# danilodjor/fault-tolerant-llm-training

Hardware: AMD Instinct MI355X
Metric: tokens/sec/GPU seq-len 2048 DP at 1/2/4/8 MI355X; checkpoint save wall-clock (s) (higher is better)
Workload: dtype bf16; 1 GPU; model=llama3-8b, global_batch=1, seq_len=2048, parallelism=dp1

## Files before the change

### csrc/kernels/gemm_w4.h

```cpp
#pragma once

#include "torch_utils.h"

#include <utility>

namespace ftw4 {


typedef int i32x4_t __attribute__((ext_vector_type(4)));

template <typename F, int... I>
__device__ __forceinline__ void sfor_impl(F&& f, std::integer_sequence<int, I...>) {
  (f(std::integral_constant<int, I>{}), ...);
}
template <int N, typename F>
__device__ __forceinline__ void sfor(F&& f) {
  sfor_impl(f, std::make_integer_sequence<int, N>{});
}

constexpr int BM = 256, BK = 64, NT = 256;
constexpr int PIECE = 1024;
constexpr int FS = 2 * PIECE;
constexpr int OPA = 32 * PIECE;
constexpr int RBA = 2 * BM;
// ... 491 lines not shown
      if (wid == 0) {
        int* fl = flags + (lane & 7);
        const bool watch = (lane & 7) < nsplit - 1;
        int v = 0;
        for (int n = 0; n < p.spin; ++n) {
          v = __hip_atomic_load(fl, __ATOMIC_RELAXED, __HIP_MEMORY_SCOPE_AGENT);
          if (__all(!watch || v != 0)) break;
          __builtin_amdgcn_s_sleep(4);
        }
        __builtin_amdgcn_fence(__ATOMIC_ACQUIRE, "agent");
        const bool miss = watch && v == 0;
        if (!miss) __hip_atomic_store(fl, 0, __ATOMIC_RELAXED, __HIP_MEMORY_SCOPE_AGENT);
        const bool any = __any(miss);
        if (lane == 0) {
          lost = any ? 1 : 0;
          if (any) __hip_atomic_fetch_add(p.err, 1, __ATOMIC_RELAXED, __HIP_MEMORY_SCOPE_AGENT);
        }
      }
      asm volatile("s_waitcnt vmcnt(0)" ::: "memory");
      __syncthreads();
      split_slot = slot - (long)ks * SLOT;
      split_lost = __builtin_amdgcn_readfirstlane(lost);
    }
  }

  barrier();
  char* wl = smem + wid * 32768;
  {
    const int lr = lane & 15, hc = lane >> 4;
#pragma unroll
    for (int i = 0; i < 8; ++i) {
      const int m = i * 16 + lr;
      float4 ps[NJ];
      if (split_slot != nullptr) {
#pragma unroll
        for (int j = 0; j < NJ; ++j) ps[j] = split_slot[(i * NJ + j) * 64];
        for (int sl = 1; sl < nsplit - 1; ++sl) {
          const float4* q = split_slot + (long)sl * (4L * 8 * NJ * 64);
#pragma unroll
          for (int j = 0; j < NJ; ++j) {
            const float4 t = q[(i * NJ + j) * 64];
            ps[j].x += t.x;
            ps[j].y += t.y;
            ps[j].z += t.z;
            ps[j].w += t.w;
          }
        }
      }
#pragma unroll
      for (int j = 0; j < NJ; ++j) {
        const int ch = 2 * j + (hc >> 1);
        f32x4_t v = acc[i][j];
        if (split_slot != nullptr) {
          v[0] = ps[j].x + v[0];
          v[1] = ps[j].y + v[1];
          v[2] = ps[j].z + v[2];
          v[3] = ps[j].w + v[3];
          if (split_lost) v = f32x4_t{__builtin_nanf(""), __builtin_nanf(""), __builtin_nanf(""), __builtin_nanf("")};
        }
        uint2 pk;
        pk.x = pk2<E>(v[0], v[1]);
        pk.y = pk2<E>(v[2], v[3]);
        *reinterpret_cast<uint2*>(wl + m * 256 + ((ch ^ (m & 15)) << 4) + (((hc ^ (m >> 3)) & 1) << 3)) = pk;
      }
    }
  }
  __builtin_amdgcn_s_waitcnt(0xc07f);
  __builtin_amdgcn_wave_barrier();
#ifdef FT_W4_PROBE
  pt3 = __builtin_amdgcn_s_memrealtime();
#endif
  const int cc = lane & 15;
  float sq = 0.f;
  if constexpr (EPI == W4_SWIGLU_BWD) {
    if (cc < 2 * NJ) {
      const int gn = n0 + wn * NW + cc * 8;
#pragma unroll
      for (int hb = 0; hb < 2; ++hb) {
        uint4 g16[16], u16[16];
#pragma unroll
        for (int q = 0; q < 16; ++q) {
          const long gm = m0 + wm * 128 + (hb * 16 + q) * 4 + (lane >> 4);
          g16[q] = *reinterpret_cast<const uint4*>(p.r + gm * p.ldr + gn);
          u16[q] = *reinterpret_cast<const uint4*>(p.r + gm * p.ldr + p.ffn + gn);
        }
#pragma unroll
        for (int q = 0; q < 16; ++q) {
          const int row = (hb * 16 + q) * 4 + (lane >> 4);
          const long gm = m0 + wm * 128 + row;
          const uint4 v = stg_swap(*reinterpret_cast<const uint4*>(wl + row * 256 + ((cc ^ (row & 15)) << 4)),
                                   (q >> 1) & 1);
          float d8[8], g8[8], u8[8], dg[8], du[8];
          unpack8e<E>(v, d8);
          unpack8e<E>(g16[q], g8);
          unpack8e<E>(u16[q], u8);
#pragma unroll
          for (int e = 0; e < 8; ++e) swiglu_grad(g8[e], u8[e], d8[e], p.exact, dg[e], du[e]);
          *reinterpret_cast<uint4*>(p.c + gm * p.ldc + gn) = pack8e<E>(dg);
          *reinterpret_cast<uint4*>(p.c + gm * p.ldc + p.ffn + gn) = pack8e<E>(du);
        }
      }
    }
  } else if (cc < 2 * NJ) {
    auto store_rows = [&](auto tail_tag) {
      constexpr bool TAIL = decltype(tail_tag)::value;
      for (int r4 = 0; r4 < 32; r4 += 4)
#pragma unroll
      for (int u = 0; u < 4; ++u) {
        const int rr = r4 + u;
        const int row = rr * 4 + (lane >> 4);
        const long gm = m0 + wm * 128 + row;
        if constexpr (TAIL) {
          if (gm >= p.M) continue;
        }
        uint4 v = stg_swap(*reinterpret_cast<const uint4*>(wl + row * 256 + ((cc ^ (row & 15)) << 4)),
                           u >> 1);
        const int gn = EPI == W4_SWIGLU ? (wn ? p.ffn : 0) + f0 + cc * 8 : n0 + wn * NW + cc * 8;
        if constexpr (EPI == W4_RES) {
          float a[8], r[8];
          unpack8e<E>(v, a);
          unpack8e<E>(*reinterpret_cast<const uint4*>(p.r + gm * p.ldr + gn), r);
#pragma unroll
          for (int q = 0; q < 8; ++q) a[q] += r[q];
          v = pack8e<E>(a);
        } else if constexpr (EPI == W4_ROPE) {
          if (gn < p.rope_cols) {
            const int pos = (int)(gm % p.rope_seq);
            const int i0 = (gn % p.rope_hd) >> 1;
            const float* cs = p.cos_t + (long)pos * (p.rope_hd >> 1) + i0;
            const float* sn = p.sin_t + (long)pos * (p.rope_hd >> 1) + i0;
            const float4 c4 = *reinterpret_cast<const float4*>(cs);
            const float4 s4 = *reinterpret_cast<const float4*>(sn);
            float a[8];
            unpack8e<E>(v, a);
            const float cv[4] = {c4.x, c4.y, c4.z, c4.w}, sv[4] = {s4.x, s4.y, s4.z, s4.w};
            float o[8];
#pragma unroll
            for (int q = 0; q < 4; ++q) {
              o[2 * q] = a[2 * q] * cv[q] - a[2 * q + 1] * sv[q];
              o[2 * q + 1] = a[2 * q] * sv[q] + a[2 * q + 1] * cv[q];
            }
            v = pack8e<E>(o);
          }
        }
        if (p.part != nullptr) {
          float a[8];
          unpack8e<E>(v, a);
#pragma unroll
          for (int q = 0; q < 8; ++q) sq = fmaf(a[q], a[q], sq);
        }
        if (!(p.dbg & 1)) *reinterpret_cast<uint4*>(p.c + gm * p.ldc + gn) = v;
      }
    };
    if (mtail)
      store_rows(std::true_type{});
    else
      store_rows(std::false_type{});
  }
  if (p.part != nullptr) {
    sq = wave_sum(sq);
    __syncthreads();
    float* red = reinterpret_cast<float*>(smem);
    if (lane == 0) red[wid] = sq;
    __syncthreads();
    if (tid == 0) p.part[tn * p.tiles_m + tm] = (red[0] + red[1]) + (red[2] + red[3]);
    if (tb == 0)
      for (int i = ntiles + tid; i < p.part_n; i += NT) p.part[i] = 0.f;
  }
  if constexpr (EPI == W4_SWIGLU) {
    __syncthreads();
    char* gl = smem + (wm * 2) * 32768;
    char* ul = smem + (wm * 2 + 1) * 32768;
    if (cc < 2 * NJ) {
      for (int r4 = 0; r4 < 16; r4 += 4)
#pragma unroll
      for (int u = 0; u < 4; ++u) {
        const int row = wn * 64 + (r4 + u) * 4 + (lane >> 4);
        const int off = row * 256 + ((cc ^ (row & 15)) << 4);
        const bool sw = u >> 1;
        float g8[8], u8[8], a8[8];
        unpack8e<E>(stg_swap(*reinterpret_cast<const uint4*>(gl + off), sw), g8);
        unpack8e<E>(stg_swap(*reinterpret_cast<const uint4*>(ul + off), sw), u8);
#pragma unroll
        for (int q = 0; q < 8; ++q) a8[q] = g8[q] * sigmoid_f(g8[q], p.exact) * u8[q];
        const uint4 av = pack8e<E>(a8);
        *reinterpret_cast<uint4*>(p.act + (m0 + wm * 128 + row) * (long)p.ffn + f0 + cc * 8) = av;
        *reinterpret_cast<uint4*>(gl + off) = stg_swap(av, sw);
      }
    }
    if (p.actT == nullptr) {
      probe_end();
      return;
    }
    __syncthreads();
    constexpr int CH = 2 * NJ;
    for (int k = tid; k < 2 * 16 * CH; k += NT) {
      const int fc = k % CH, tg = (k / CH) % 16, hf = k / (16 * CH);
      const char* al = smem + (hf * 2) * 32768;
      uint16_t e[8][8];
#pragma unroll
      for (int i = 0; i < 8; ++i) {
        const int row = tg * 8 + i;
        const uint4 v = stg_swap(*reinterpret_cast<const uint4*>(al + row * 256 + ((fc ^ (row & 15)) << 4)), tg & 1);
        const uint32_t wv[4] = {v.x, v.y, v.z, v.w};
#pragma unroll
        for (int q = 0; q < 4; ++q) {
          e[i][2 * q] = (uint16_t)(wv[q] & 0xffffu);
          e[i][2 * q + 1] = (uint16_t)(wv[q] >> 16);
        }
      }
      bf16_t* dst = p.actT + (long)(f0 + fc * 8) * p.M + m0 + hf * 128 + tg * 8;
#pragma unroll
      for (int j = 0; j < 8; ++j) {
        uint4 o;
        o.x = e[0][j] | ((uint32_t)e[1][j] << 16);
        o.y = e[2][j] | ((uint32_t)e[3][j] << 16);
        o.z = e[4][j] | ((uint32_t)e[5][j] << 16);
        o.w = e[6][j] | ((uint32_t)e[7][j] << 16);
        *reinterpret_cast<uint4*>(dst + (long)j * p.M) = o;
      }
    }
  }
  probe_end();
}

template <class E, int NJ, bool AT, bool BT>
void launch_nj(const W4Args& p, int epi, hipStream_t st) {
  const dim3 g(p.tiles_m * p.tiles_n * (p.splits > 1 ? p.splits : 1));
  if constexpr (!AT && !BT) {
    if (epi == W4_ROPE) {
      hipLaunchKernelGGL((gemm_w4_kernel<E, NJ, W4_ROPE, false, false>), g, dim3(NT), 0, st, p);
      return;
    }
    if (epi == W4_SWIGLU) {
      hipLaunchKernelGGL((gemm_w4_kernel<E, NJ, W4_SWIGLU, false, false>), g, dim3(NT), 0, st, p);
      return;
    }
  }
  if constexpr (!AT && BT) {
    if (epi == W4_SWIGLU_BWD) {
      hipLaunchKernelGGL((gemm_w4_kernel<E, NJ, W4_SWIGLU_BWD, false, true>), g, dim3(NT), 0, st, p);
      return;
    }
  }
  TORCH_CHECK(epi == W4_STORE || epi == W4_RES, "gemm_w4: epilogue ", epi, " not built for this layout");
  if (epi == W4_RES)
    hipLaunchKernelGGL((gemm_w4_kernel<E, NJ, W4_RES, AT, BT>), g, dim3(NT), 0, st, p);
  else
    hipLaunchKernelGGL((gemm_w4_kernel<E, NJ, W4_STORE, AT, BT>), g, dim3(NT), 0, st, p);
}

template <bool AT, bool BT>
void launch_l(at::ScalarType st_, int nj, const W4Args& p, int epi, hipStream_t st) {
  FT_DISPATCH_E16(st_, {
    switch (nj) {
      case 8: launch_nj<E, 8, AT, BT>(p, epi, st); break;
      case 7: launch_nj<E, 7, AT, BT>(p, epi, st); break;
      case 6: launch_nj<E, 6, AT, BT>(p, epi, st); break;
      default: launch_nj<E, 4, AT, BT>(p, epi, st); break;
    }
  });
}

void launch_fwd(at::ScalarType st_, int nj, const W4Args& p, int epi, hipStream_t st);
void launch_dx(at::ScalarType st_, int nj, const W4Args& p, int epi, hipStream_t st);
void launch_dw(at::ScalarType st_, int nj, const W4Args& p, int epi, hipStream_t st);

}
```

### fault_tolerant_llm_training_amd/models/llama.py

```python
from __future__ import annotations

from dataclasses import dataclass, replace
from typing import Optional

import torch
import torch.utils.checkpoint
import torch.nn as nn

from ..ops import functional as Fx
from .flat import FlatParamSpace


@dataclass
class TransformerModelArgs:

    dim: int = 4096
    n_layers: int = 32
    n_heads: int = 32
    n_kv_heads: Optional[int] = None
    multiple_of: int = 256
    ffn_dim_multiplier: Optional[float] = None
    norm_eps: float = 1e-5
    rope_theta: float = 10000
    norm_type: str = "rmsnorm"
    seq_len: int = 2048
    vocab_size: int = -1

    @property
    def kv_heads(self) -> int:
        return self.n_heads if self.n_kv_heads is None else self.n_kv_heads

    @property
    def head_dim(self) -> int:
        return self.dim // self.n_heads

    @property
    def ffn_hidden(self) -> int:
        hidden = int(2 * (4 * self.dim) / 3)
        if self.ffn_dim_multiplier is not None:
            hidden = int(self.ffn_dim_multiplier * hidden)
        return self.multiple_of * ((hidden + self.multiple_of - 1) // self.multiple_of)


PRESETS = {
    "llama3-8b": dict(dim=4096, n_layers=32, n_heads=32, n_kv_heads=8, ffn_dim_multiplier=1.3,
                      multiple_of=1024, rope_theta=500000),
    "gpt2-small": dict(dim=768, n_layers=12, n_heads=12, n_kv_heads=12, multiple_of=256,
                       rope_theta=10000),
    "gpt2-medium": dict(dim=1024, n_layers=24, n_heads=16, n_kv_heads=16, multiple_of=256,
                        rope_theta=10000),
    "tiny": dict(dim=256, n_layers=2, n_heads=4, n_kv_heads=2, multiple_of=64, rope_theta=10000),
}


def model_args_for(preset: str, vocab_size: int, seq_len: int, **overrides) -> TransformerModelArgs:
    if preset not in PRESETS:
        raise ValueError(f"unknown model preset {preset!r}; choose from {sorted(PRESETS)}")
    cfg = dict(PRESETS[preset])
    cfg.update(overrides)
    return TransformerModelArgs(vocab_size=vocab_size, seq_len=seq_len, **cfg)


def rope_tables(head_dim: int, end: int, theta: float):
    freqs = 1.0 / (theta ** (torch.arange(0, head_dim, 2)[: (head_dim // 2)].float() / head_dim))
    t = torch.arange(end, device=freqs.device)
    freqs = torch.outer(t, freqs).float()
    cis = torch.polar(torch.ones_like(freqs), freqs)
    return cis.real.contiguous(), cis.imag.contiguous()


class _Weight(nn.Module):

    def __init__(self, *shape):
        super().__init__()
        self.weight = nn.Parameter(torch.empty(*shape, device="meta"))


class Attention(nn.Module):
    def __init__(self, a: TransformerModelArgs):
        super().__init__()
        self.n_heads, self.n_kv_heads, self.head_dim = a.n_heads, a.kv_heads, a.head_dim
        self.wq = _Weight(a.n_heads * a.head_dim, a.dim)
        self.wk = _Weight(a.kv_heads * a.head_dim, a.dim)
        self.wv = _Weight(a.kv_heads * a.head_dim, a.dim)
        self.wo = _Weight(a.dim, a.n_heads * a.head_dim)
        self.wqkv = None
        self.wqkv_sink = None


class FeedForward(nn.Module):
    def __init__(self, a: TransformerModelArgs):
        super().__init__()
        h = a.ffn_hidden
        self.w1 = _Weight(h, a.dim)
        self.w2 = _Weight(a.dim, h)
        self.w3 = _Weight(h, a.dim)
        self.w13 = None
        self.w13_sink = None


class TransformerBlock(nn.Module):
    def __init__(self, layer_id: int, a: TransformerModelArgs):
        super().__init__()
        self.layer_id = layer_id
        self.attention = Attention(a)
        self.feed_forward = FeedForward(a)
        self.attention_norm = _Weight(a.dim)
        self.ffn_norm = _Weight(a.dim)
        self.eps = a.norm_eps
        self.layernorm = a.norm_type == "layernorm"
        self.attn_keep = Fx.AttentionKeep()

    def forward(self, h, d, cos, sin, seq_len, gen=None, doc=None):
        at, ff = self.attention, self.feed_forward
        sk = lambda p: getattr(p, "_ft_sink", None)
        if d is None:
            xn = Fx.norm(h, self.attention_norm.weight, sk(self.attention_norm.weight), self.eps, self.layernorm)
        else:
            h, xn = Fx.add_norm(h, d, self.attention_norm.weight, sk(self.attention_norm.weight), self.eps,
                                self.layernorm)
        o = Fx.qkv_rope_attention(xn, at.wqkv, at.wqkv_sink, cos, sin, seq_len, at.n_heads, at.n_kv_heads,
                                  at.head_dim, self.attn_keep if gen is not None else None, -1 if gen is None else gen,
                                  doc)
        da = Fx.linear(o.view(*h.shape[:-1], -1), at.wo.weight, sk(at.wo.weight))
        h, hn = Fx.add_norm(h, da, self.ffn_norm.weight, sk(self.ffn_norm.weight), self.eps, self.layernorm)
        return h, Fx.feed_forward(hn, ff.w13, ff.w2.weight, ff.w13_sink, sk(ff.w2.weight))


class Transformer(nn.Module):
    def __init__(self, model_args: TransformerModelArgs):
        super().__init__()
        a = model_args
        self.model_args = a
        self.vocab_size = a.vocab_size
        self.n_layers = a.n_layers
        self.tok_embeddings = _Weight(a.vocab_size, a.dim)
        cos, sin = rope_tables(a.head_dim, a.seq_len, a.rope_theta)
        self.register_buffer("rope_cos", cos, persistent=False)
        self.register_buffer("rope_sin", sin, persistent=False)
        self.layers = nn.ModuleDict({str(i): TransformerBlock(i, a) for i in range(a.n_layers)})
        self.norm = _Weight(a.dim)
        self.output = _Weight(a.vocab_size, a.dim)
        self.flat: Optional[FlatParamSpace] = None
        self.gate = None
        self._ranges = None
        self.recompute_layers = 0
        self.recompute_attention = False
        self._gen = 0
        self.doc_bos: Optional[int] = None

    def set_document_mask(self, bos_id: Optional[int]) -> None:
        self.doc_bos = None if bos_id is None else int(bos_id)

    def set_activation_checkpointing(self, n_layers: int, recompute_attention: bool = False) -> None:
        self.recompute_layers = self.n_layers if n_layers < 0 else min(int(n_layers), self.n_layers)
        self.recompute_attention = bool(recompute_attention)

    def flat_layout(self):
        names = ["tok_embeddings.weight"]
        for i in range(self.n_layers):
            p = f"layers.{i}."
            names += [p + "attention_norm.weight", p + "attention.wq.weight", p + "attention.wk.weight",
                      p + "attention.wv.weight", p + "attention.wo.weight", p + "ffn_norm.weight",
                      p + "feed_forward.w1.weight", p + "feed_forward.w3.weight", p + "feed_forward.w2.weight"]
        names += ["norm.weight", "output.weight"]
        return names

    def materialize(self, device, dtype=torch.bfloat16, seed: int = 1234) -> "Transformer":
        self.flat = FlatParamSpace(self, self.flat_layout(), device, dtype)
        self.rope_cos = self.rope_cos.to(device)
        self.rope_sin = self.rope_sin.to(device)
        for layer in self.layers.values():
            at, ff = layer.attention, layer.feed_forward
            i = layer.layer_id
            at.wqkv, at.wqkv_sink = self.flat.fused(
                [f"layers.{i}.attention.wq.weight", f"layers.{i}.attention.wk.weight", f"layers.{i}.attention.wv.weight"])
            ff.w13, ff.w13_sink = self.flat.fused(
                [f"layers.{i}.feed_forward.w1.weight", f"layers.{i}.feed_forward.w3.weight"])
        self._ranges = self._param_ranges()
        self.init_weights(seed)
        return self

    def _param_ranges(self):
        sl = self.flat.slots

        def span(prefix):
            ss = [s for n, s in sl.items() if n.startswith(prefix)]
            return min(s.offset for s in ss), max(s.offset + s.numel for s in ss)

        emb = span("tok_embeddings.")
        layers = [span(f"layers.{i}.") for i in range(self.n_layers)]
        lo_n, hi_n = span("norm.")
        lo_o, hi_o = span("output.")
        return emb, layers, (min(lo_n, lo_o), max(hi_n, hi_o))

    def _wait(self, rng):
        if self.gate is not None:
            self.gate.wait(*rng)

    @torch.no_grad()
    def init_weights(self, seed: int = 1234):
        dev = self.flat.device
        gen = torch.Generator(device=dev)
        for idx, (name, p) in enumerate(self.named_parameters()):
            gen.manual_seed(seed * 1000003 + idx)
            if name == "tok_embeddings.weight":
                p.normal_(0.0, 1.0, generator=gen)
            elif p.dim() == 1:
                p.fill_(1.0)
            else:
                bound = 1.0 / (p.shape[1] ** 0.5)
                p.uniform_(-bound, bound, generator=gen)

    def sinks_in_backward_order(self):
        out = []
        for layer in self.layers.values():
            out += [layer.attention.wqkv_sink, layer.feed_forward.w13_sink]
        return out

    def forward(self, tokens: torch.Tensor, labels: Optional[torch.Tensor] = None,
                inv_count: Optional[torch.Tensor] = None):
        B, S = tokens.shape
        sk = lambda p: getattr(p, "_ft_sink", None)
        emb_r, layer_r, final_r = self._ranges
        self._wait(emb_r)
        h = Fx.embedding(tokens, self.tok_embeddings.weight, sk(self.tok_embeddings.weight))
        cos, sin = self.rope_cos, self.rope_sin
        doc = None if self.doc_bos is None else Fx.doc_bounds(tokens, self.doc_bos)
        d = None
        self._gen += 1
        gen = None if self.recompute_attention else self._gen
        for i, layer in enumerate(self.layers.values()):
            self._wait(layer_r[i])
            if i < self.recompute_layers and torch.is_grad_enabled():
                h, d = torch.utils.checkpoint.checkpoint(layer, h, d, cos, sin, S, gen, doc, use_reentrant=False)
            else:
                h, d = layer(h, d, cos, sin, S, None, doc)
        self._wait(final_r)
        a = self.model_args
        ln = a.norm_type == "layernorm"
        if d is None:
            h = Fx.norm(h, self.norm.weight, sk(self.norm.weight), a.norm_eps, ln)
        else:
            _, h = Fx.add_norm(h, d, self.norm.weight, sk(self.norm.weight), a.norm_eps, ln)
        if labels is None:
            return Fx.linear(h, self.output.weight, sk(self.output.weight))
        if inv_count is None:
            n = (labels != Fx.IGNORE_INDEX).sum().clamp(min=1)
            inv_count = (1.0 / n.float()).to(h.device)
        return Fx.lm_head_cross_entropy(h, self.output.weight, labels, inv_count, sk(self.output.weight))

    @torch.no_grad()
    def evaluate(self, tokens: torch.Tensor, labels: torch.Tensor, acc: torch.Tensor) -> torch.Tensor:
        B, S = tokens.shape
        emb_r, layer_r, final_r = self._ranges
        self._wait(emb_r)
        h = Fx.embedding(tokens, self.tok_embeddings.weight, None)
        cos, sin = self.rope_cos, self.rope_sin
        doc = None if self.doc_bos is None else Fx.doc_bounds(tokens, self.doc_bos)
        d = None
        self._gen += 1
        for i, layer in enumerate(self.layers.values()):
            self._wait(layer_r[i])
            h, d = layer(h, d, cos, sin, S, None, doc)
        self._wait(final_r)
        a = self.model_args
        ln = a.norm_type == "layernorm"
        if d is None:
            h = Fx.norm(h, self.norm.weight, None, a.norm_eps, ln)
        else:
            _, h = Fx.add_norm(h, d, self.norm.weight, None, a.norm_eps, ln)
        return Fx.lm_head_eval(h, self.output.weight, labels, acc)

    def num_params(self) -> int:
        return sum(p.numel() for p in self.parameters())


def build_model(args: TransformerModelArgs, device, dtype=torch.bfloat16, seed: int = 1234) -> Transformer:
    return Transformer(args).materialize(device, dtype, seed)


PEAK_FLOPS = {torch.bfloat16: 2.5e15, torch.float16: 2.5e15, torch.float32: 157.3e12, torch.float64: 78.6e12}


def flops_per_token(a: TransformerModelArgs, seq_len: int) -> float:
    d, L, hd = a.dim, a.n_layers, a.head_dim
    per_layer = d * (a.n_heads * hd) + 2 * d * (a.kv_heads * hd) + (a.n_heads * hd) * d + 3 * d * a.ffn_hidden
    n_mm = L * per_layer + d * a.vocab_size
    attn = L * 2 * 2 * seq_len * a.n_heads * hd / 2
    return 6 * n_mm + 3 * attn
```

### fault_tolerant_llm_training_amd/ops/functional.py

```python
from __future__ import annotations

import collections
import functools
import os
from typing import Optional

import torch
import torch.nn.functional as F

from .._native import kernels, native
from .grad_sink import GradSink

IGNORE_INDEX = -100

_BLAS_ONLY = os.environ.get("FT_GEMM_BLAS", "0") == "1"
_W4_FWD = True
_W4_BWD = os.environ.get("FT_W4_BWD", "1") != "0"
_W4_DTYPES = (torch.bfloat16, torch.float16)
_F32_MFMA = os.environ.get("FT_F32_MFMA", "1") != "0"


def set_f32_mfma(on: bool) -> None:
    global _F32_MFMA
    _F32_MFMA = bool(on)
# ... 201 lines not shown
        ctx.wshape = weight.shape
        if native(weight):
            return kernels().embedding_fwd(tokens.contiguous(), weight)
        return F.embedding(tokens, weight)

    @staticmethod
    def backward(ctx, dy):
        (tokens,) = ctx.saved_tensors
        sink = ctx.sink
        dy = dy.contiguous()
        if sink is not None and sink.gather is not None:
            if sink.defer:
                sink.stash.append((tokens.reshape(-1), dy.reshape(-1, dy.shape[-1])))
                return None, None, None
            if sink.stash:
                tokens = torch.cat([t for t, _ in sink.stash] + [tokens.reshape(-1)])
                dy = torch.cat([g for _, g in sink.stash] + [dy.reshape(-1, dy.shape[-1])])
                sink.stash = []
            tokens, dy = sink.gather(tokens, dy)
        if native(dy):
            if sink is None:
                dw = torch.zeros(ctx.wshape, dtype=dy.dtype, device=dy.device)
                kernels().embedding_bwd_(dy, tokens.contiguous(), dw, False)
                return None, dw, None
            part = sink.part if (sink.part is not None and not sink.accumulate) else None
            kernels().embedding_bwd_(dy, tokens.contiguous(), sink.buf, sink.accumulate, part)
            if part is not None:
                sink.sq_done = True
            sink.ready()
            return None, None, None
        dw = torch.zeros(ctx.wshape, dtype=torch.float32, device=dy.device)
        if dy.is_cuda:
            dw.index_put_((tokens.reshape(-1),), dy.reshape(-1, ctx.wshape[1]).float(), accumulate=True)
        else:
            dw.index_add_(0, tokens.reshape(-1), dy.reshape(-1, ctx.wshape[1]).float())
        return None, _write_weight_grad(sink, dw.to(dy.dtype)), None


def embedding(tokens, weight, sink=None):
    return EmbeddingFn.apply(tokens, weight, sink)


def norm_reference(x: torch.Tensor, w: torch.Tensor, eps: float, layernorm: bool) -> torch.Tensor:
    xf = x.float()
    if layernorm:
        xf = xf - xf.mean(-1, keepdim=True)
    n = xf * torch.rsqrt(xf.pow(2).mean(-1, keepdim=True) + eps)
    return n.type_as(x) * w


class NormFn(torch.autograd.Function):
    @staticmethod
    def forward(ctx, x, weight, sink, eps, layernorm):
        ctx.sink, ctx.eps, ctx.ln = sink, eps, layernorm
        if native(x):
            xc = x.contiguous()
            y, rstd, mean = kernels().norm_fwd(xc, weight, eps, layernorm)
            ctx.save_for_backward(xc, weight, rstd, mean)
            return y
        ctx.save_for_backward(x, weight)
        return norm_reference(x, weight, eps, layernorm)

    @staticmethod
    def backward(ctx, dy):
        sink = ctx.sink
        if native(dy):
            x, w, rstd, mean = ctx.saved_tensors
            if sink is not None:
                return norm_bwd_into_sink(dy.contiguous(), x, w, rstd, mean, sink), None, None, None, None
            dw = torch.empty_like(w)
            dx = kernels().norm_bwd(dy.contiguous(), x, w, rstd, mean, dw, None, False)
            return dx, dw, None, None, None
        x, w = ctx.saved_tensors
        with torch.enable_grad():
            xr = x.detach().requires_grad_(True)
            wr = w.detach().requires_grad_(True)
            y = norm_reference(xr, wr, ctx.eps, ctx.ln)
            dx, dw = torch.autograd.grad(y, (xr, wr), dy)
        return dx, _write_weight_grad(sink, dw), None, None, None


def norm(x, weight, sink=None, eps: float = 1e-5, layernorm: bool = False):
    return NormFn.apply(x, weight, sink, eps, layernorm)


class AddNormFn(torch.autograd.Function):

    @staticmethod
    def forward(ctx, x, d, weight, sink, eps, layernorm):
        ctx.sink, ctx.eps, ctx.ln = sink, eps, layernorm
        if native(x):
            y, rstd, mean, h = kernels().add_norm_fwd(x.contiguous(), d.contiguous(), weight, eps, layernorm)
            ctx.save_for_backward(h, weight, rstd, mean)
            return h, y
        h = x + d
        ctx.save_for_backward(h, weight)
        return h, norm_reference(h, weight, eps, layernorm)

    @staticmethod
    def backward(ctx, dh, dy):
        sink = ctx.sink
        if native(dy):
            h, w, rstd, mean = ctx.saved_tensors
            dres = dh.contiguous() if dh is not None else None
            if sink is not None:
                g = norm_bwd_into_sink(dy.contiguous(), h, w, rstd, mean, sink, dres)
                return g, g, None, None, None, None
            buf = torch.empty_like(w)
            g = kernels().norm_bwd(dy.contiguous(), h, w, rstd, mean, buf, dres, False)
            return g, g, buf, None, None, None
        h, w = ctx.saved_tensors
        with torch.enable_grad():
            hr = h.detach().requires_grad_(True)
            wr = w.detach().requires_grad_(True)
            y = norm_reference(hr, wr, ctx.eps, ctx.ln)
            g, dw = torch.autograd.grad(y, (hr, wr), dy)
        if dh is not None:
            g = g + dh
        return g, g, _write_weight_grad(sink, dw), None, None, None


def add_norm(x, d, weight, sink=None, eps: float = 1e-5, layernorm: bool = False):
    return AddNormFn.apply(x, d, weight, sink, eps, layernorm)


class LinearFn(torch.autograd.Function):
    @staticmethod
    def forward(ctx, x, weight, sink, residual):
        K = x.shape[-1]
        N = weight.shape[0]
        x2 = x.reshape(-1, K)
        y = mm_fwd(x2, weight, residual)
        ctx.sink = sink
        ctx.has_res = residual is not None
        ctx.xshape = x.shape
        ctx.save_for_backward(x2, weight)
        return y.view(*x.shape[:-1], N)

    @staticmethod
    def backward(ctx, dy):
        x2, w = ctx.saved_tensors
        N = w.shape[0]
        dy2 = dy.reshape(-1, N)
        dw = None
        dw = weight_grad_async(dy2, x2, ctx.sink)
        dx = mm_dx(dy2, w).view(ctx.xshape)
        return dx, dw, None, (dy if ctx.has_res else None)


def linear(x, weight, sink=None, residual=None):
    return LinearFn.apply(x, weight, sink, residual)


def swiglu_reference(gu: torch.Tensor) -> torch.Tensor:
    g, u = gu.chunk(2, dim=-1)
    return F.silu(g) * u


class SwiGLUFn(torch.autograd.Function):
    @staticmethod
    def forward(ctx, gu):
        ctx.save_for_backward(gu)
        if native(gu):
            return kernels().swiglu_fwd(gu.contiguous())
        return swiglu_reference(gu)

    @staticmethod
    def backward(ctx, da):
        (gu,) = ctx.saved_tensors
        if native(da):
            return kernels().swiglu_bwd(da.contiguous(), gu.contiguous())
        with torch.enable_grad():
            x = gu.detach().requires_grad_(True)
            (dx,) = torch.autograd.grad(swiglu_reference(x), (x,), da)
        return dx


def swiglu(gu):
    return SwiGLUFn.apply(gu)


_W4_SWIGLU = True


def set_w4_swiglu(on: bool) -> None:
    global _W4_SWIGLU
    _W4_SWIGLU = bool(on)


def _ffn_w4t_ok(x2: torch.Tensor, w13: torch.Tensor, w2: torch.Tensor) -> bool:
    if not (_W4_SWIGLU and _W4_FWD and _W4_BWD and w13.is_contiguous() and w2.is_contiguous()):
        return False
    T, D = x2.shape
    F = w2.shape[1]
    if T % 256 or D % 128:
        return False
    nj = _swiglu_nj(T, F)
    if nj == 0 or (T // 256) * (F // (16 * nj)) < _W4_MIN_WGS:
        return False
    return (w4_route(T, F, D, False, True, x2, w2) and w4_route(2 * F, D, T, True, True, x2, w13)
            and w4_route(D, F, T, True, True, x2, w2) and w4_route(T, D, 2 * F, False, True, x2, w13))


@functools.lru_cache(maxsize=64)
def _swiglu_nj(T: int, F: int) -> int:
    return int(kernels().gemm_swiglu_pick(T, F))


class FeedForwardW4Fn(torch.autograd.Function):

    @staticmethod
    def forward(ctx, x, w13, w2, sink13, sink2):
        K_ = kernels()
        D = x.shape[-1]
        x2 = x.reshape(-1, D).contiguous()
        gu, a, _ = K_.gemm_swiglu_w4(x2, w13, False)
        y = mm_fwd(a, w2)
        ctx.sinks = (sink13, sink2)
        ctx.xshape = x.shape
        ctx.save_for_backward(x2, gu, a, w13, w2)
        return y.view(*x.shape[:-1], w2.shape[0])

    @staticmethod
    def backward(ctx, dy):
        x2, gu, a, w13, w2 = ctx.saved_tensors
        sink13, sink2 = ctx.sinks
        dy2 = dy.reshape(-1, w2.shape[0]).contiguous()
        dw2 = weight_grad_async(dy2, a, sink2)
        dgu = kernels().gemm_swiglu_bwd_w4(dy2, w2, gu, 0)
        dw13 = weight_grad_async(dgu, x2, sink13)
        dx = mm_dx(dgu, w13).view(ctx.xshape)
        return dx, dw13, dw2, None, None


class FeedForwardFn(torch.autograd.Function):

    @staticmethod
    def forward(ctx, x, w13, w2, sink13, sink2):
        K_ = kernels()
        D = x.shape[-1]
        x2 = x.reshape(-1, D)
        gu = mm_fwd(x2, w13)
        a = K_.swiglu_fwd(gu)
        y = mm_fwd(a, w2)
        ctx.sinks = (sink13, sink2)
        ctx.xshape = x.shape
        ctx.save_for_backward(x2, gu, a, w13, w2)
        return y.view(*x.shape[:-1], w2.shape[0])

    @staticmethod
    def backward(ctx, dy):
        x2, gu, a, w13, w2 = ctx.saved_tensors
        sink13, sink2 = ctx.sinks
        dy2 = dy.reshape(-1, w2.shape[0]).contiguous()
        dw2 = weight_grad_async(dy2, a, sink2)
        dgu = kernels().swiglu_bwd(mm_dx(dy2, w2), gu)
        dw13 = weight_grad_async(dgu, x2, sink13)
        dx = mm_dx(dgu, w13).view(ctx.xshape)
        return dx, dw13, dw2, None, None


def feed_forward(x, w13, w2, sink13=None, sink2=None):
    if native(x):
        T, D = x.numel() // x.shape[-1], x.shape[-1]
        if _ffn_w4t_ok(x.reshape(T, D), w13, w2):
            return FeedForwardW4Fn.apply(x, w13, w2, sink13, sink2)
        return FeedForwardFn.apply(x, w13, w2, sink13, sink2)
    return linear(swiglu(linear(x, w13, sink13)), w2, sink2)


_HEAD_CHUNK_MB = float(os.environ.get("FT_HEAD_CHUNK_MB", "1024"))


def _head_rows(T: int, V: int) -> int:
    rows = int(_HEAD_CHUNK_MB * 2**20) // (2 * V)
    rows = max(256, rows // 256 * 256)
    return min(T, rows)


def _dx_into(out: torch.Tensor, dy2: torch.Tensor, w: torch.Tensor) -> None:
    mm_dx(dy2, w, out)


def _head_fwd(h2: torch.Tensor, w: torch.Tensor) -> torch.Tensor:
    return mm_fwd(h2.contiguous(), w)


class LMHeadCrossEntropyFn(torch.autograd.Function):

    @staticmethod
    def forward(ctx, h, weight, sink, labels, inv_count):
        D = h.shape[-1]
        h2 = h.reshape(-1, D)
        lab = labels.reshape(-1)
        ctx.sink = sink
        ctx.hshape = h.shape
        ctx.native = native(h)
        if not ctx.native:
            logits = torch.mm(h2, weight.t())
            loss = F.cross_entropy(logits.float(), lab, reduction="sum", ignore_index=IGNORE_INDEX) * inv_count
            ctx.save_for_backward(h2, weight, lab, inv_count)
            return loss
        K_ = kernels()
        h2 = h2.contiguous()
        lab = lab.contiguous()
        T, V = h2.shape[0], weight.shape[0]
        rows = _head_rows(T, V)
        need = ctx.needs_input_grad[0] or ctx.needs_input_grad[1] or sink is not None
        fused = need and not (sink is not None and sink.accumulate)
        ctx.fused = fused
        ctx.rows = rows
        inv = inv_count.float().reshape(1).contiguous()
        one = torch.ones(1, dtype=torch.float32, device=h.device)
        dh = torch.empty_like(h2) if fused else None
        dw = None
        if fused:
            dw = sink.buf.view(V, D) if sink is not None else torch.empty_like(weight)
        losses, lses = [], []
        for c, r0 in enumerate(range(0, T, rows)):
            hc, lc = h2[r0 : r0 + rows], lab[r0 : r0 + rows]
            logits = _head_fwd(hc, weight)
            lr, lse = K_.xent_fwd(logits, lc, IGNORE_INDEX)
            losses.append(lr)
            if fused:
                K_.xent_bwd_(logits, lc, lse, one, inv, IGNORE_INDEX)
                _dx_into(dh[r0 : r0 + rows], logits, weight)
                _dw_into(dw, logits, hc, c > 0, sink if r0 + rows >= T else None)
            else:
                lses.append(lse)
            del logits
        loss = (losses[0] if len(losses) == 1 else torch.cat(losses)).sum() * inv_count
        if fused:
            ctx.save_for_backward(dh, dw if sink is None else None)
        else:
            ctx.save_for_backward(h2, weight, lab, inv, torch.cat(lses))
        return loss

    @staticmethod
    def backward(ctx, g):
        sink = ctx.sink
        if not ctx.native:
            h2, w, lab, inv_count = ctx.saved_tensors
            with torch.enable_grad():
                hr = h2.detach().requires_grad_(True)
                wr = w.detach().requires_grad_(True)
                logits = torch.mm(hr, wr.t())
                loss = F.cross_entropy(logits.float(), lab, reduction="sum", ignore_index=IGNORE_INDEX) * inv_count
                dh, dw = torch.autograd.grad(loss, (hr, wr), g)
            return dh.view(ctx.hshape), _write_weight_grad(sink, dw), None, None, None
        K_ = kernels()
        gf = g.detach().float().reshape(1).contiguous()
        if ctx.fused:
            dh, dw = ctx.saved_tensors
            K_.scale_by_(dh, gf)
            if sink is not None:
                K_.scale_by_(sink.buf, gf)
                if sink.sq_done:
                    sink.part.mul_(gf * gf)
                sink.ready()
                return dh.view(ctx.hshape), None, None, None, None
            K_.scale_by_(dw, gf)
            return dh.view(ctx.hshape), dw, None, None, None
        h2, w, lab, inv, lse = ctx.saved_tensors
        T, D = h2.shape
        V = w.shape[0]
        rows = ctx.rows
        dh = torch.empty_like(h2)
        dw = sink.buf.view(V, D) if sink is not None else torch.empty_like(w)
        acc0 = sink.accumulate if sink is not None else False
        for c, r0 in enumerate(range(0, T, rows)):
            hc, lc = h2[r0 : r0 + rows], lab[r0 : r0 + rows]
            logits = _head_fwd(hc, w)
            K_.xent_bwd_(logits, lc, lse[r0 : r0 + rows].contiguous(), gf, inv, IGNORE_INDEX)
            _dx_into(dh[r0 : r0 + rows], logits, w)
            _dw_into(dw, logits, hc, acc0 or c > 0, sink if r0 + rows >= T else None)
            del logits
        if sink is not None:
            sink.ready()
            return dh.view(ctx.hshape), None, None, None, None
        return dh.view(ctx.hshape), dw, None, None, None


def lm_head_cross_entropy(h, weight, labels, inv_count, sink=None):
    return LMHeadCrossEntropyFn.apply(h, weight, sink, labels, inv_count)

# ... 35 lines not shown
```

### fault_tolerant_llm_training_amd/ops/routing.py

```python
from . import attention as A
from . import functional as Fx


class _Spec:

    def __init__(self, *shape, dtype, cuda=True):
        self.shape, self.dtype, self.is_cuda = tuple(shape), dtype, cuda

    def is_contiguous(self):
        return True


def _name(kernel, M, N, K, a_t, b_t):
    if kernel != "w4":
        return {"f32": "f32 mfma", "blas": "hipBLASLt"}[kernel]
    nj, sp = Fx._w4_plan(M, N, K, a_t, b_t)
    return f"w4 {32 * nj}" + (f" x{sp}" if sp > 1 else "")


def routing_table(margs, dtype, tokens: int = 2048, cuda: bool = True) -> dict:
    T, D, V = tokens, margs.dim, margs.vocab_size
    hd, Hq, Hkv, Fh = margs.head_dim, margs.n_heads, margs.kv_heads, margs.ffn_hidden
    W = (Hq + 2 * Hkv) * hd
    sp = lambda *s: _Spec(*s, dtype=dtype, cuda=cuda)
    x, wqkv, wo, w13, w2, head = sp(T, D), sp(W, D), sp(D, Hq * hd), sp(2 * Fh, D), sp(D, Fh), sp(V, D)

    def fwd(xx, w):
        return _name(Fx.fwd_kernel(xx, w), xx.shape[0], w.shape[0], xx.shape[1], False, False)

    def dx(Tn, w):
        N, K = w.shape
        return _name(Fx.dx_kernel(sp(Tn, N), w), Tn, K, N, False, True)

    def dw(Tn, w):
        N, K = w.shape
        return _name(Fx.dw_kernel(sp(Tn, N), sp(Tn, K)), N, K, Tn, True, True)

    t = {}
    t["qkv fwd"] = "w4 qkv+rope" if A._qkv_rope_ok(x, wqkv, hd) else fwd(x, wqkv)
    t["qkv dX"], t["qkv dW"] = dx(T, wqkv), dw(T, wqkv)
    t["wo fwd"], t["wo dX"], t["wo dW"] = fwd(sp(T, Hq * hd), wo), dx(T, wo), dw(T, wo)
    if cuda and Fx._ffn_w4t_ok(x, w13, w2):
        t["w13 fwd"], t["w2 dX"] = "w4 swiglu", "w4 swiglu-bwd"
    else:
        t["w13 fwd"], t["w2 dX"] = fwd(x, w13), dx(T, w2)
    t["w13 dX"], t["w13 dW"] = dx(T, w13), dw(T, w13)
    t["w2 fwd"], t["w2 dW"] = fwd(sp(T, Fh), w2), dw(T, w2)
    rows = Fx._head_rows(T, V)
    t["head fwd"], t["head dX"], t["head dW"] = fwd(sp(rows, D), head), dx(rows, head), dw(rows, head)
    return t
```

Measured before the change: 20780 tokens/s (whole job, sum over GPUs).

## Fuse residual add into W4 down-projection GEMM epilogue and hoist next-layer norm

Adds a residual-add epilogue path to the W4 GEMM store so the FFN down-projection writes h + FFN(x) directly. The block then computes the next layer's attention norm inside a fused autograd function, which removes the separate add_norm kernel and its read/write of the residual stream. The same fusion for the wo projection exists but is off by default. In exchange the forward signature and checkpointing path get more complex, and the epilogue does extra global loads of the residual per tile.

```diff
diff --git a/csrc/kernels/gemm_w4.h b/csrc/kernels/gemm_w4.h
--- a/csrc/kernels/gemm_w4.h
+++ b/csrc/kernels/gemm_w4.h
@@ -667,8 +667,42 @@
         if (!(p.dbg & 1)) *reinterpret_cast<uint4*>(p.c + gm * p.ldc + gn) = v;
       }
     };
+    auto store_rows_res = [&]() {
+      const int gn = n0 + wn * NW + cc * 8;
+#pragma unroll
+      for (int hb = 0; hb < 2; ++hb) {
+        uint4 r16[16];
+#pragma unroll
+        for (int q = 0; q < 16; ++q) {
+          const long gm = m0 + wm * 128 + (hb * 16 + q) * 4 + (lane >> 4);
+          r16[q] = *reinterpret_cast<const uint4*>(p.r + gm * p.ldr + gn);
+        }
+#pragma unroll
+        for (int q = 0; q < 16; ++q) {
+          const int row = (hb * 16 + q) * 4 + (lane >> 4);
+          const long gm = m0 + wm * 128 + row;
+          uint4 v = stg_swap(*reinterpret_cast<const uint4*>(wl + row * 256 + ((cc ^ (row & 15)) << 4)),
+                             (q >> 1) & 1);
+          float a[8], r[8];
+          unpack8e<E>(v, a);
+          unpack8e<E>(r16[q], r);
+#pragma unroll
+          for (int e = 0; e < 8; ++e) a[e] += r[e];
+          v = pack8e<E>(a);
+          if (p.part != nullptr) {
+            float s[8];
+            unpack8e<E>(v, s);
+#pragma unroll
+            for (int e = 0; e < 8; ++e) sq = fmaf(s[e], s[e], sq);
+          }
+          if (!(p.dbg & 1)) *reinterpret_cast<uint4*>(p.c + gm * p.ldc + gn) = v;
+        }
+      }
+    };
     if (mtail)
       store_rows(std::true_type{});
+    else if constexpr (EPI == W4_RES)
+      store_rows_res();
     else
       store_rows(std::false_type{});
   }
diff --git a/fault_tolerant_llm_training_amd/models/llama.py b/fault_tolerant_llm_training_amd/models/llama.py
--- a/fault_tolerant_llm_training_amd/models/llama.py
+++ b/fault_tolerant_llm_training_amd/models/llama.py
@@ -111,10 +111,12 @@
         self.layernorm = a.norm_type == "layernorm"
         self.attn_keep = Fx.AttentionKeep()
 
-    def forward(self, h, d, cos, sin, seq_len, gen=None, doc=None):
+    def forward(self, h, d, cos, sin, seq_len, gen=None, doc=None, xn=None, next_norm=None):
         at, ff = self.attention, self.feed_forward
         sk = lambda p: getattr(p, "_ft_sink", None)
-        if d is None:
+        if xn is not None:
+            pass
+        elif d is None:
             xn = Fx.norm(h, self.attention_norm.weight, sk(self.attention_norm.weight), self.eps, self.layernorm)
         else:
             h, xn = Fx.add_norm(h, d, self.attention_norm.weight, sk(self.attention_norm.weight), self.eps,
@@ -122,9 +124,18 @@
         o = Fx.qkv_rope_attention(xn, at.wqkv, at.wqkv_sink, cos, sin, seq_len, at.n_heads, at.n_kv_heads,
                                   at.head_dim, self.attn_keep if gen is not None else None, -1 if gen is None else gen,
                                   doc)
-        da = Fx.linear(o.view(*h.shape[:-1], -1), at.wo.weight, sk(at.wo.weight))
-        h, hn = Fx.add_norm(h, da, self.ffn_norm.weight, sk(self.ffn_norm.weight), self.eps, self.layernorm)
-        return h, Fx.feed_forward(hn, ff.w13, ff.w2.weight, ff.w13_sink, sk(ff.w2.weight))
+        o = o.view(*h.shape[:-1], -1)
+        if Fx.native(o) and Fx.linear_res_ok(o.view(-1, o.shape[-1]), at.wo.weight):
+            h, hn = Fx.linear_add_norm(o, at.wo.weight, h, self.ffn_norm.weight, sk(at.wo.weight),
+                                       sk(self.ffn_norm.weight), self.eps, self.layernorm)
+        else:
+            da = Fx.linear(o, at.wo.weight, sk(at.wo.weight))
+            h, hn = Fx.add_norm(h, da, self.ffn_norm.weight, sk(self.ffn_norm.weight), self.eps, self.layernorm)
+        if next_norm is not None and Fx.native(hn) and Fx.ffn_res_ok(hn.view(-1, hn.shape[-1]), ff.w13, ff.w2.weight):
+            h, xn = Fx.feed_forward_add_norm(hn, ff.w13, ff.w2.weight, h, next_norm, ff.w13_sink, sk(ff.w2.weight),
+                                             sk(next_norm), self.eps, self.layernorm)
+            return h, None, xn
+        return h, Fx.feed_forward(hn, ff.w13, ff.w2.weight, ff.w13_sink, sk(ff.w2.weight)), None
 
 
 class Transformer(nn.Module):
@@ -144,6 +155,7 @@
         self.flat: Optional[FlatParamSpace] = None
         self.gate = None
         self._ranges = None
+        self._norm_names = None
         self.recompute_layers = 0
         self.recompute_attention = False
         self._gen = 0
@@ -178,6 +190,7 @@
             ff.w13, ff.w13_sink = self.flat.fused(
                 [f"layers.{i}.feed_forward.w1.weight", f"layers.{i}.feed_forward.w3.weight"])
         self._ranges = self._param_ranges()
+        self._norm_names = [f"layers.{i}.attention_norm.weight" for i in range(self.n_layers)] + ["norm.weight"]
         self.init_weights(seed)
         return self
 
@@ -193,6 +206,14 @@
         lo_n, hi_n = span("norm.")
         lo_o, hi_o = span("output.")
         return emb, layers, (min(lo_n, lo_o), max(hi_n, hi_o))
+
+    def _next_norm(self, i, layers):
+        w = layers[i + 1].attention_norm.weight if i + 1 < len(layers) else self.norm.weight
+        if self.gate is not None and self.flat is not None:
+            s = self.flat.slots.get(self._norm_names[i + 1]) if self._norm_names else None
+            if s is not None:
+                self.gate.wait(s.offset, s.offset + s.numel)
+        return w
 
     def _wait(self, rng):
         if self.gate is not None:
@@ -227,19 +248,24 @@
         h = Fx.embedding(tokens, self.tok_embeddings.weight, sk(self.tok_embeddings.weight))
         cos, sin = self.rope_cos, self.rope_sin
         doc = None if self.doc_bos is None else Fx.doc_bounds(tokens, self.doc_bos)
-        d = None
+        d = xn = None
         self._gen += 1
         gen = None if self.recompute_attention else self._gen
-        for i, layer in enumerate(self.layers.values()):
+        layers = list(self.layers.values())
+        for i, layer in enumerate(layers):
             self._wait(layer_r[i])
+            nxt = self._next_norm(i, layers)
             if i < self.recompute_layers and torch.is_grad_enabled():
-                h, d = torch.utils.checkpoint.checkpoint(layer, h, d, cos, sin, S, gen, doc, use_reentrant=False)
+                h, d, xn = torch.utils.checkpoint.checkpoint(layer, h, d, cos, sin, S, gen, doc, xn, nxt,
+                                                             use_reentrant=False)
             else:
-                h, d = layer(h, d, cos, sin, S, None, doc)
+                h, d, xn = layer(h, d, cos, sin, S, None, doc, xn, nxt)
         self._wait(final_r)
         a = self.model_args
         ln = a.norm_type == "layernorm"
-        if d is None:
+        if xn is not None:
+            h = xn
+        elif d is None:
             h = Fx.norm(h, self.norm.weight, sk(self.norm.weight), a.norm_eps, ln)
         else:
             _, h = Fx.add_norm(h, d, self.norm.weight, sk(self.norm.weight), a.norm_eps, ln)
@@ -258,15 +284,18 @@
         h = Fx.embedding(tokens, self.tok_embeddings.weight, None)
         cos, sin = self.rope_cos, self.rope_sin
         doc = None if self.doc_bos is None else Fx.doc_bounds(tokens, self.doc_bos)
-        d = None
+        d = xn = None
         self._gen += 1
-        for i, layer in enumerate(self.layers.values()):
+        layers = list(self.layers.values())
+        for i, layer in enumerate(layers):
             self._wait(layer_r[i])
-            h, d = layer(h, d, cos, sin, S, None, doc)
+            h, d, xn = layer(h, d, cos, sin, S, None, doc, xn, self._next_norm(i, layers))
         self._wait(final_r)
         a = self.model_args
         ln = a.norm_type == "layernorm"
-        if d is None:
+        if xn is not None:
+            h = xn
+        elif d is None:
             h = Fx.norm(h, self.norm.weight, None, a.norm_eps, ln)
         else:
             _, h = Fx.add_norm(h, d, self.norm.weight, None, a.norm_eps, ln)
diff --git a/fault_tolerant_llm_training_amd/ops/functional.py b/fault_tolerant_llm_training_amd/ops/functional.py
--- a/fault_tolerant_llm_training_amd/ops/functional.py
+++ b/fault_tolerant_llm_training_amd/ops/functional.py
@@ -377,6 +377,66 @@
     return LinearFn.apply(x, weight, sink, residual)
 
 
+_W4_RESIDUAL = True
+_W4_RESIDUAL_WO = False
+
+
+def set_w4_residual(on: bool, wo: Optional[bool] = None) -> None:
+    global _W4_RESIDUAL, _W4_RESIDUAL_WO
+    _W4_RESIDUAL = bool(on)
+    if wo is not None:
+        _W4_RESIDUAL_WO = bool(wo)
+
+
+def _res_fwd_w4(T: int, N: int, K: int, x, w) -> bool:
+    return _W4_RESIDUAL and _kernel(_W4_FWD, w.is_contiguous(), T, N, K, False, False, x, w) == "w4"
+
+
+def linear_res_ok(x2, w) -> bool:
+    return _W4_RESIDUAL_WO and _res_fwd_w4(x2.shape[0], w.shape[0], x2.shape[1], x2, w)
+
+
+def ffn_res_ok(x2, w13, w2) -> bool:
+    return (x2.is_cuda and _ffn_w4t_ok(x2, w13, w2)
+            and _res_fwd_w4(x2.shape[0], w2.shape[0], w2.shape[1], x2, w2))
+
+
+def _norm_bwd_res(ctx, saved, dh, dy):
+    h1, nw, rstd, mean = saved
+    dres = dh.contiguous() if dh is not None else None
+    if ctx.norm_sink is not None:
+        return norm_bwd_into_sink(dy.contiguous(), h1, nw, rstd, mean, ctx.norm_sink, dres), None
+    buf = torch.empty_like(nw)
+    return kernels().norm_bwd(dy.contiguous(), h1, nw, rstd, mean, buf, dres, False), buf
+
+
+class LinearAddNormFn(torch.autograd.Function):
+
+    @staticmethod
+    def forward(ctx, x, weight, h, norm_w, sink, norm_sink, eps, layernorm):
+        K, N = x.shape[-1], weight.shape[0]
+        x2 = x.reshape(-1, K).contiguous()
+        h1 = kernels().gemm_nt_w4(x2, weight, None, h.reshape(-1, N).contiguous(), 0, 0).view(h.shape)
+        y, rstd, mean = kernels().norm_fwd(h1, norm_w, eps, layernorm)
+        ctx.sink, ctx.norm_sink, ctx.xshape = sink, norm_sink, x.shape
+        ctx.save_for_backward(h1, norm_w, rstd, mean, x2, weight)
+        return h1, y
+
+    @staticmethod
+    def backward(ctx, dh, dy):
+        saved = ctx.saved_tensors
+        x2, w = saved[4:]
+        g, dnw = _norm_bwd_res(ctx, saved[:4], dh, dy)
+        dy2 = g.reshape(-1, w.shape[0])
+        dw = weight_grad_async(dy2, x2, ctx.sink)
+        dx = mm_dx(dy2, w).view(ctx.xshape)
+        return dx, dw, g, dnw, None, None, None, None
+
+
+def linear_add_norm(x, weight, h, norm_w, sink=None, norm_sink=None, eps: float = 1e-5, layernorm: bool = False):
+    return LinearAddNormFn.apply(x, weight, h, norm_w, sink, norm_sink, eps, layernorm)
+
+
 def swiglu_reference(gu: torch.Tensor) -> torch.Tensor:
     g, u = gu.chunk(2, dim=-1)
     return F.silu(g) * u
@@ -456,6 +516,39 @@
         dw13 = weight_grad_async(dgu, x2, sink13)
         dx = mm_dx(dgu, w13).view(ctx.xshape)
         return dx, dw13, dw2, None, None
+
+
+class FeedForwardW4AddNormFn(torch.autograd.Function):
+
+    @staticmethod
+    def forward(ctx, x, w13, w2, h, norm_w, sink13, sink2, norm_sink, eps, layernorm):
+        K_ = kernels()
+        D = x.shape[-1]
+        x2 = x.reshape(-1, D).contiguous()
+        gu, a, _ = K_.gemm_swiglu_w4(x2, w13, False)
+        h1 = K_.gemm_nt_w4(a, w2, None, h.reshape(-1, w2.shape[0]).contiguous(), 0, 0).view(h.shape)
+        y, rstd, mean = K_.norm_fwd(h1, norm_w, eps, layernorm)
+        ctx.sinks, ctx.norm_sink, ctx.xshape = (sink13, sink2), norm_sink, x.shape
+        ctx.save_for_backward(h1, norm_w, rstd, mean, x2, gu, a, w13, w2)
+        return h1, y
+
+    @staticmethod
+    def backward(ctx, dh, dy):
+        saved = ctx.saved_tensors
+        x2, gu, a, w13, w2 = saved[4:]
+        sink13, sink2 = ctx.sinks
+        g, dnw = _norm_bwd_res(ctx, saved[:4], dh, dy)
+        dy2 = g.reshape(-1, w2.shape[0])
+        dw2 = weight_grad_async(dy2, a, sink2)
+        dgu = kernels().gemm_swiglu_bwd_w4(dy2, w2, gu, 0)
+        dw13 = weight_grad_async(dgu, x2, sink13)
+        dx = mm_dx(dgu, w13).view(ctx.xshape)
+        return dx, dw13, dw2, g, dnw, None, None, None, None, None
+
+
+def feed_forward_add_norm(x, w13, w2, h, norm_w, sink13=None, sink2=None, norm_sink=None, eps: float = 1e-5,
+                          layernorm: bool = False):
+    return FeedForwardW4AddNormFn.apply(x, w13, w2, h, norm_w, sink13, sink2, norm_sink, eps, layernorm)
 
 
 class FeedForwardFn(torch.autograd.Function):
diff --git a/fault_tolerant_llm_training_amd/ops/routing.py b/fault_tolerant_llm_training_amd/ops/routing.py
--- a/fault_tolerant_llm_training_amd/ops/routing.py
+++ b/fault_tolerant_llm_training_amd/ops/routing.py
@@ -16,6 +16,14 @@
         return {"f32": "f32 mfma", "blas": "hipBLASLt"}[kernel]
     nj, sp = Fx._w4_plan(M, N, K, a_t, b_t)
     return f"w4 {32 * nj}" + (f" x{sp}" if sp > 1 else "")
+
+
+def residual_table(margs, dtype, tokens: int = 2048, cuda: bool = True) -> dict:
+    T, D, Fh = tokens, margs.dim, margs.ffn_hidden
+    sp = lambda *s: _Spec(*s, dtype=dtype, cuda=cuda)
+    x, wo, w13, w2 = sp(T, D), sp(D, margs.n_heads * margs.head_dim), sp(2 * Fh, D), sp(D, Fh)
+    return {"wo": bool(cuda and Fx.linear_res_ok(sp(T, margs.n_heads * margs.head_dim), wo)),
+            "w2": bool(cuda and Fx.ffn_res_ok(x, w13, w2))}
 
 
 def routing_table(margs, dtype, tokens: int = 2048, cuda: bool = True) -> dict:
```

New measurement: 20770 tokens/s (whole job, sum over GPUs). About the same (-0.1%).
